# RozDavid/UnScene3D

Hardware: AMD Instinct MI355X
Metric: training scenes/sec (Res16UNet34C+Mask3D, 150k voxels) (higher is better)
Workload: dtype f32

## Files before the change

include/usc3d.h:

```cpp
#ifndef USC3D_H
#define USC3D_H

#include <stdint.h>

#ifdef __cplusplus
extern "C" {
#endif

typedef void* usc_stream_t;

enum usc_status {
  USC_OK = 0,
  USC_ERR_ARG = -1,
  USC_ERR_LAUNCH = -2,
  USC_ERR_RANGE = -3
};

const char* usc_last_error(void);
int usc_abi_version(void);
const char* usc_build_info(void);
int usc_device_count(void);


int usc_voxel_floor_f64(const double* xyz, int64_t n, double voxel_size,
                        int32_t* coords_out, usc_stream_t s);

int usc_voxel_floor_f64_host(const double* xyz, int64_t n, double voxel_size,
                             int32_t* coords_out);
int usc_unique_coords_host(const int32_t* coords, int64_t n, int32_t d,
                           int64_t* unique_idx, int64_t* inverse,
                           int64_t* n_out);

int64_t usc_coordmap_capacity(int64_t n);
int64_t usc_coordmap_ws_bytes(int64_t n);

int usc_coordmap_build(const int32_t* coords, int64_t n, int32_t quant,
                       uint64_t* table_keys, int32_t* table_vals, int64_t cap,
                       int64_t* unique_idx, int64_t* inverse,
                       int32_t* out_coords, int64_t* n_out,
                       void* ws, int64_t ws_bytes, usc_stream_t s);

int usc_morton_cell_ids(const int32_t* coords, int64_t n, int32_t shift,
                        int32_t lo_x, int32_t lo_y, int32_t lo_z,
                        int32_t bits_per_axis, int64_t* ids, usc_stream_t s);


int usc_kernel_map_cube(const int32_t* coords, int64_t n, int32_t tensor_stride,
                        int32_t ksize, const uint64_t* table_keys,
                        const int32_t* table_vals, int64_t cap, int32_t* nbr,
                        usc_stream_t s);

int usc_kernel_map_down2(const int32_t* fine_coords, int64_t n_fine,
                         int32_t tensor_stride, const int64_t* parent,
                         const int32_t* coarse_coords, int64_t n_coarse,
                         int32_t* nbr2, uint8_t* kidx, usc_stream_t s);

int64_t usc_rulebook_ws_bytes(int64_t K, int64_t n_out);
int usc_rulebook_compact(const int32_t* nbr, int64_t K, int64_t n_out,
                         int32_t* in_idx, int32_t* out_idx, int64_t* koff,
                         void* ws, int64_t ws_bytes, usc_stream_t s);


int usc_weight_transpose(const float* W, int32_t K, int32_t cin, int32_t cout,
                         int32_t mirror, float* out, usc_stream_t s);

int usc_spconv_plan(int32_t kind, int64_t n, int32_t cin, int32_t cout,
                    int32_t K);
int64_t usc_rowsort_ws_bytes(int32_t K, int64_t n_out);
int usc_rowsort_build(const int32_t* nbr, int32_t K, int64_t n_out,
                      int32_t* perm, uint32_t* tile_mask, void* ws,
                      int64_t ws_bytes, usc_stream_t s);
int64_t usc_spconv_sorted_ws_bytes(int64_t n_out, int32_t cin, int32_t cout,
                                   int32_t K);
int usc_spconv_sorted_gemm(const float* in, int64_t n_in, int32_t cin,
                           const float* W, int32_t K, int32_t cout,
                           const int32_t* nbr, const int32_t* perm,
                           const uint32_t* tile_mask, int64_t n_out,
                           const float* bias, float* out, int32_t accumulate,
                           int32_t w_transposed, void* ws, int64_t ws_bytes,
                           usc_stream_t s);
int usc_spconv_sorted_gemm_ex(const float* in, int64_t n_in, int32_t cin,
                              const float* W, int32_t K, int32_t cout,
                              const int32_t* nbr, const int32_t* perm,
                              const uint32_t* tile_mask, int64_t n_out,
                              const float* bias, float* out, int32_t accumulate,
                              int32_t w_transposed, void* ws, int64_t ws_bytes,
                              int32_t* slices_left, usc_stream_t s);
int usc_group_reduce(const float* partial, int32_t G, int64_t n, int32_t c,
                     const float* bias, int32_t accumulate, float* out,
                     usc_stream_t s);

int64_t usc_spconv_gather_gemm_ws_bytes(int64_t n_out, int32_t cin,
                                        int32_t cout, int32_t K);
int usc_spconv_gather_gemm(const float* in, int64_t n_in, int32_t cin,
                           const float* W, int32_t K, int32_t cout,
                           const int32_t* nbr, int64_t n_out,
                           const float* bias, float* out, int32_t accumulate, int32_t w_transposed,
                           void* ws, int64_t ws_bytes, usc_stream_t s);

int usc_spconv_pairs_gemm(const float* in, int32_t cin, const float* W,
                          int32_t K, int32_t cout, const int32_t* rows_in,
                          const int32_t* rows_out, const int64_t* koff,
                          int64_t P_capacity, float* out, usc_stream_t s);

int usc_cast_bf16(const float* in, int64_t n, uint16_t* out, usc_stream_t s);
int usc_spconv_pack_w_bf16(const float* W, int32_t K, int32_t cin, int32_t cout,
                           uint16_t* Wp, usc_stream_t s);
int64_t usc_spconv_gather_gemm_bf16_ws_bytes(int64_t n_out, int32_t cin,
                                             int32_t cout, int32_t K);
int usc_spconv_gather_gemm_bf16(const uint16_t* in, int64_t n_in, int32_t cin,
                                const uint16_t* Wp, int32_t K, int32_t cout,
                                const int32_t* nbr, int64_t n_out,
                                const float* bias, float* out, int32_t accumulate,
                                void* ws, int64_t ws_bytes, usc_stream_t s);

int usc_split_bf16_rows(const float* in, int64_t rows, int32_t c, int32_t P,
                        uint16_t* out, usc_stream_t s);
int usc_split_bf16(const float* in, int64_t n, int32_t P, uint16_t* out,
                   usc_stream_t s);
int usc_spconv_pack_w_split(const float* W, int32_t K, int32_t cin, int32_t cout,
// ... 477 lines not shown
```

unscene3d_amd/_lib.py:

```python
from __future__ import annotations

import ctypes as C
import os

import torch

_HERE = os.path.dirname(os.path.abspath(__file__))
LIB_PATH = os.environ.get("USC3D_LIB") or os.path.join(_HERE, "libusc3d_hip.so")

_p = C.c_void_p
_i32 = C.c_int32
_i64 = C.c_int64
_f64 = C.c_double
_f32 = C.c_float

class KMap(C.Structure):
    _fields_ = [("nbr", _p), ("perm", _p), ("tile_mask", _p), ("pair_in", _p), ("pair_out", _p), ("koff", _p),
                ("n_in", _i64), ("n_out", _i64), ("pair_capacity", _i64), ("K", _i32), ("reserved", _i32)]


class BNDesc(C.Structure):
    _fields_ = [("gamma", _p), ("beta", _p), ("running_mean", _p), ("running_var", _p), ("num_batches_tracked", _p),
                ("eps", _f32), ("momentum", _f32), ("c", _i32), ("training", _i32)]


_kp = C.POINTER(KMap)
_bp = C.POINTER(BNDesc)


class Step(C.Structure):
    _fields_ = [("op", _i32), ("kind", _i32), ("cin", _i32), ("cout", _i32), ("relu", _i32),
                ("dx_accumulate", _i32), ("dW_accumulate", _i32), ("dbn_accumulate", _i32), ("defer_wgrad", _i32),
                ("accumulate", _i32),
                ("map", _p), ("bn", _p),
                ("x", _p), ("W", _p), ("residual", _p), ("y", _p), ("stats", _p), ("out", _p),
                ("dout", _p), ("dy", _p), ("dres", _p), ("dx", _p), ("dW", _p), ("dgamma", _p), ("dbeta", _p),
                ("a", _p), ("b", _p), ("dst", _p), ("dst2", _p), ("n", _i64), ("ca", _i32), ("cb", _i32),
                ("split_planes", _i32), ("reserved", _i32)]


_sp = C.POINTER(Step)
STEP_UNIT_FWD, STEP_UNIT_BWD, STEP_CAT, STEP_SPLIT, STEP_ADD, STEP_UNIT_FWD_BF16 = 0, 1, 2, 3, 4, 5

SIGNATURES = {
    "usc_last_error": (C.c_char_p, []),
    "usc_abi_version": (C.c_int, []),
    "usc_build_info": (C.c_char_p, []),
    "usc_device_count": (C.c_int, []),
    "usc_voxel_floor_f64": (C.c_int, [_p, _i64, _f64, _p, _p]),
    "usc_voxel_floor_f64_host": (C.c_int, [_p, _i64, C.c_double, _p]),
    "usc_unique_coords_host": (C.c_int, [_p, _i64, _i32, _p, _p, _p]),
    "usc_coordmap_capacity": (_i64, [_i64]),
    "usc_coordmap_ws_bytes": (_i64, [_i64]),
    "usc_coordmap_build": (C.c_int, [_p, _i64, _i32, _p, _p, _i64, _p, _p, _p, _p, _p, _i64, _p]),
    "usc_morton_cell_ids": (C.c_int, [_p, _i64, _i32, _i32, _i32, _i32, _i32, _p, _p]),
    "usc_kernel_map_cube": (C.c_int, [_p, _i64, _i32, _i32, _p, _p, _i64, _p, _p]),
    "usc_kernel_map_down2": (C.c_int, [_p, _i64, _i32, _p, _p, _i64, _p, _p, _p]),
    "usc_rulebook_ws_bytes": (_i64, [_i64, _i64]),
    "usc_rulebook_compact": (C.c_int, [_p, _i64, _i64, _p, _p, _p, _p, _i64, _p]),
    "usc_weight_transpose": (C.c_int, [_p, _i32, _i32, _i32, _i32, _p, _p]),
    "usc_spconv_plan": (C.c_int, [_i32, _i64, _i32, _i32, _i32]),
    "usc_spconv_gather_gemm_ws_bytes": (_i64, [_i64, _i32, _i32, _i32]),
    "usc_spconv_gather_gemm": (C.c_int, [_p, _i64, _i32, _p, _i32, _i32, _p, _i64, _p, _p, _i32, _i32, _p, _i64, _p]),
    "usc_rowsort_ws_bytes": (_i64, [_i32, _i64]),
    "usc_rowsort_build": (C.c_int, [_p, _i32, _i64, _p, _p, _p, _i64, _p]),
    "usc_spconv_sorted_ws_bytes": (_i64, [_i64, _i32, _i32, _i32]),
    "usc_spconv_sorted_gemm": (C.c_int, [_p, _i64, _i32, _p, _i32, _i32, _p, _p, _p, _i64, _p, _p, _i32, _i32, _p, _i64, _p]),
    "usc_spconv_sorted_gemm_ex": (C.c_int, [_p, _i64, _i32, _p, _i32, _i32, _p, _p, _p, _i64, _p, _p, _i32, _i32, _p, _i64, _p, _p]),
    "usc_group_reduce": (C.c_int, [_p, _i32, _i64, _i32, _p, _i32, _p, _p]),
    "usc_bn_tile_max_rows": (C.c_int64, []),
    "usc_bn_plan": (_i64, [_i64, _i32, _i32]),
    "usc_bn_tile_ok": (C.c_int, [_i64, _i32]),
    "usc_bn_tile_ws_bytes": (C.c_int64, [_i32]),
    "usc_bn_tile_forward": (C.c_int, [_p, _i32, _p, _i64, _i32, _p, _p, _f32, _f32, _p, _p, _p, _p, _p, _p, _p, _p, _i32, _p,
                                      _p, _i64, _p]),
    "usc_bn_tile_backward": (C.c_int, [_p, _i32, _i32, _p, _p, _p, _p, _p, _p, _i64, _i32, _i32, _i32, _p, _p, _p, _p, _p,
                                       _i64, _p]),
    "usc_spconv_pairs_gemm": (C.c_int, [_p, _i32, _p, _i32, _i32, _p, _p, _p, _i64, _p, _p]),
    "usc_cast_bf16": (C.c_int, [_p, _i64, _p, _p]),
    "usc_spconv_pack_w_bf16": (C.c_int, [_p, _i32, _i32, _i32, _p, _p]),
    "usc_spconv_gather_gemm_bf16_ws_bytes": (_i64, [_i64, _i32, _i32, _i32]),
    "usc_spconv_gather_gemm_bf16": (C.c_int, [_p, _i64, _i32, _p, _i32, _i32, _p, _i64, _p, _p, _i32, _p, _i64, _p]),
    "usc_split_bf16_rows": (C.c_int, [_p, _i64, _i32, _i32, _p, _p]),
    "usc_split_bf16": (C.c_int, [_p, _i64, _i32, _p, _p]),
    "usc_spconv_pack_w_split": (C.c_int, [_p, _i32, _i32, _i32, _i32, _i32, _p, _p]),
    "usc_spconv_gather_gemm_split_ws_bytes": (_i64, [_i64, _i32, _i32, _i32, _i32]),
    "usc_spconv_gather_gemm_split": (C.c_int, [_p, _i64, _i32, _p, _i32, _i32, _i32, _p, _i64, _p, _p, _i32, _p, _i64, _p]),
    "usc_spconv_wgrad_ws_bytes": (_i64, [_i32, _i32, _i32]),
    "usc_spconv_wgrad": (C.c_int, [_p, _i32, _p, _i32, _i32, _p, _p, _p, _i64, _p, _i32, _p, _i64, _p]),
    "usc_spconv_wgrad_ws_bytes_rows": (_i64, [_i32, _i32, _i32, _i64]),
    "usc_step_size": (_i32, []),
    "usc_program_ws_bytes": (_i64, [_sp, _i32]),
    "usc_program_run": (C.c_int, [_sp, _i32, _i32, _p, _i64, _p]),
    "usc_spconv_wgrad_group_max": (_i32, []),
    "usc_spconv_wgrad_grid_limit": (None, [_i32]),
    "usc_spconv_wgrad_group_ok": (C.c_int, [_i32, _i32, _i32, _i32, _i64]),
    "usc_spconv_wgrad_group": (C.c_int, [_i32, _p, _p, _p, _i32, _i32, _i32, _p, _p, _p, _i64, _i32, _p]),
    "usc_spconv_wgrad_table_ws_bytes": (_i64, [_i32, _i32, _i32]),
    "usc_spconv_wgrad_table": (C.c_int, [_p, _i32, _p, _i32, _p, _i32, _i64, _p, _i32, _p, _i64, _p]),
    "usc_set_wgrad_lane": (C.c_int, [_p, _p, _i64, _i64]),
    "usc_wgrad_lane_join": (C.c_int, [_p]),
    "usc_wgrad_lane_hold": (C.c_int, [_i32, _i64, _i64, _p]),
    "usc_wgrad_lane_holding": (_i32, []),
    "usc_launch_stats_begin": (C.c_int, [_p, _i64, _p]),
    "usc_launch_stats_end": (_i64, [_p, _i64]),
    "usc_wall_clock_khz": (_i64, []),
    "usc_conv_ws_bytes": (_i64, [_kp, _i32, _i32, _i32]),
    "usc_unit_ws_bytes": (_i64, [_kp, _i32, _i32, _i32]),
    "usc_conv_forward": (C.c_int, [_kp, _i32, _p, _i32, _p, _i32, _p, _p, _p, _i64, _p]),
    "usc_conv_backward": (C.c_int, [_kp, _i32, _p, _i32, _p, _i32, _p, _p, _i32, _p, _i32, _p, _i64, _p]),
    "usc_bn_eval_stats": (C.c_int, [_p, _p, _p, _p, _f32, _i32, _p, _p, _p, _p, _p]),
    "usc_conv_bn_act_forward": (C.c_int, [_kp, _i32, _p, _i32, _p, _i32, _bp, _p, _i32, _p, _p, _p, _p, _i64, _p]),
    "usc_unit_bf16_ws_bytes": (_i64, [_kp, _i32, _i32, _i32]),
    "usc_conv_bn_act_forward_bf16": (C.c_int, [_kp, _i32, _p, _i32, _p, _i32, _bp, _p, _i32, _p, _p, _p, _p, _i64, _p]),
    "usc_unit_split_ws_bytes": (_i64, [_kp, _i32, _i32, _i32, _i32]),
    "usc_conv_bn_act_forward_split": (C.c_int, [_kp, _i32, _p, _i32, _p, _i32, _i32, _bp, _p, _i32, _p, _p, _p, _p, _i64, _p]),
# ... 144 lines not shown
```

unscene3d_amd/csrc/common.h:

```cpp
#pragma once
#include <hip/hip_runtime.h>
#include <stdint.h>
#include <stdio.h>
#include <string.h>

#include "../../include/usc3d.h"

namespace usc {

constexpr int kWave = 64;

void set_error(const char* fmt, ...);

#define USC_REQUIRE(cond, ...)                   \
  do {                                           \
    if (!(cond)) {                               \
      ::usc::set_error(__VA_ARGS__);             \
      return USC_ERR_ARG;                        \
    }                                            \
  } while (0)

#define USC_CHECK_LAUNCH(name)                                                  \
  do {                                                                          \
    hipError_t e__ = hipGetLastError();                                         \
// ... 35 lines not shown
  k ^= k >> 30; k *= 0xbf58476d1ce4e5b9ull;
  k ^= k >> 27; k *= 0x94d049bb133111ebull;
  k ^= k >> 31;
  return k;
}

__host__ __device__ inline int floor_quant(int c, int q) {
  int d = c / q;
  if ((c % q != 0) && ((c < 0) != (q < 0))) --d;
  return d * q;
}

#if defined(__HIPCC__)
__device__ inline int table_lookup(const uint64_t* __restrict__ keys,
                                   const int32_t* __restrict__ vals, int64_t cap,
                                   uint64_t key) {
  uint64_t slot = hash_key(key) & (uint64_t)(cap - 1);
  for (;;) {
    uint64_t k = keys[slot];
    if (k == key) return vals[slot];
    if (k == kEmptyKey) return -1;
    slot = (slot + 1) & (uint64_t)(cap - 1);
  }
}

__device__ inline int lane_id() { return threadIdx.x & 63; }

__device__ inline int wave_reduce_add(int v) {
#pragma unroll
  for (int o = 32; o > 0; o >>= 1) v += __shfl_xor(v, o, 64);
  return v;
}
__device__ inline float wave_reduce_addf(float v) {
#pragma unroll
  for (int o = 32; o > 0; o >>= 1) v += __shfl_xor(v, o, 64);
  return v;
}
__device__ inline double wave_reduce_addd(double v) {
#pragma unroll
  for (int o = 32; o > 0; o >>= 1) v += __shfl_xor(v, o, 64);
  return v;
}
__device__ inline int wave_inclusive_scan(int v) {
  const int l = lane_id();
#pragma unroll
  for (int o = 1; o < 64; o <<= 1) {
    int t = __shfl_up(v, o, 64);
    if (l >= o) v += t;
  }
  return v;
}
#endif

int spconv_up_table(const int32_t* nbr2, int32_t K, int64_t n_coarse, int64_t n_fine, int32_t* inv, hipStream_t st);

}
```

unscene3d_amd/csrc/spconv.hip:

```cpp
#include "common.h"

#include <stdlib.h>

#include <vector>

namespace usc {

typedef float f32x16 __attribute__((ext_vector_type(16)));

#define MFMA32(a, b, c) __builtin_amdgcn_mfma_f32_32x32x2f32((a), (b), (c), 0, 0, 0)

struct GemmParams {
  const float* in;
  const float* W;
  const int32_t* nbr;
  const float* bias;
  float* out;
  int64_t n_out;
  int cin, cout, K;
  int accumulate;
  int G;
  int TM;
  int wt1;
  const int32_t* rows_in;
// ... 891 lines not shown
  const int64_t total = per * K;
  for (int64_t j = (int64_t)blockIdx.x * blockDim.x + threadIdx.x; j < total; j += (int64_t)gridDim.x * blockDim.x) {
    const int k = (int)(j / per);
    const int64_t rem = j - (int64_t)k * per;
    const int co = (int)(rem / cin), ci = (int)(rem - (int64_t)co * cin);
    const int ks = mirror ? (K - 1 - k) : k;
    out[j] = W[(int64_t)ks * per + (int64_t)ci * cout + co];
  }
}

__global__ void weight_pack_kernel(const float* __restrict__ W, int K, int cin, int cout, int NB, int wt,
                                   float* __restrict__ out) {
  const int64_t total = (int64_t)K * cin * cout;
  const int nq = cin >> 3, BN = NB * 32;
  for (int64_t e = (int64_t)blockIdx.x * blockDim.x + threadIdx.x; e < total; e += (int64_t)gridDim.x * blockDim.x) {
    int64_t r = e;
    const int j = (int)(r & 3); r >>= 2;
    const int ln = (int)(r & 63); r >>= 6;
    const int nb = (int)(r % NB); r /= NB;
    const int q = (int)(r % nq); r /= nq;
    const int k = (int)(r % K);
    const int cb = (int)(r / K);
    const int i = ln & 31, h = ln >> 5;
    const int c = 8 * q + 4 * h + j, n = cb * BN + NB * i + nb;
    out[e] = wt ? W[((int64_t)(K - 1 - k) * cout + n) * cin + c] : W[((int64_t)k * cin + c) * cout + n];
  }
}

static int wgrad_splits(int K, int cin, int cout, int NB, int64_t n_rows) {
  const int64_t tiles = (int64_t)K * ceil_div(cin, 32) * ceil_div(cout, NB * 32);
  const int target = (K > 1 && n_rows >= (int64_t)2 << 20) ? 4096 : 2048;
  int64_t S = ceil_div(target, tiles);
  const int64_t by_rows = n_rows / 2048 + 1;
  if (S > by_rows) S = by_rows;
  if (S > 64) S = 64;
  if (S < 1) S = 1;
  return (int)S;
}
static int wgrad_full_nb(int cb) { return (cb % 3 == 0) ? 3 : (cb % 4 == 0 ? 4 : (cb % 2 == 0 ? 2 : 1)); }
static int wgrad_full_ct(int ctiles, int NBf) {
  if (NBf == 3 && ctiles % 3 != 0 && ctiles % 4 == 0) return 4;
  return (ctiles % 3 == 0 && NBf * 3 <= 9) ? 3 : ((ctiles % 4 == 0 && NBf * 4 <= 9) ? 4 : ((ctiles % 2 == 0 && NBf * 2 <= 9) ? 2 : 1));
}
static int64_t wgrad_full_splits(int K, int ctiles, int cb, int CT, int NBf, int64_t n_rows) {
  const int64_t blocks_per_split = (int64_t)K * (ctiles / CT) * (cb / NBf);
  const int64_t tgt = (K > 1 && n_rows >= (int64_t)2 << 20) ? 2048 : 512;
  int64_t S = tgt / blocks_per_split;
  const int64_t by_rows = n_rows / (K > 1 ? 4096 : 256) + 1;
  if (S > by_rows) S = by_rows;
  if (S > 64) S = 64;
  if (S < 1) S = 1;
  return S;
}
static int pick_nb(int cout) {
  if (cout <= 32) return 1;
  if (cout <= 64) return 2;
  if (cout % 128 == 0) return 4;
  if (cout % 96 == 0) return 3;
  return 4;
}

struct GemmPlan { int NB; int G; bool aligned; int TM; };
constexpr int64_t kTargetWaves = 3072;

static bool stem_form(bool has_table, int cin, int cout, int K) {
  return has_table && cin >= 1 && cin <= 4 && cout == 32 && K >= 1 && K <= 32;
}

static GemmPlan plan_table(int64_t n_out, int cin, int cout, int K) {
  GemmPlan pl{pick_nb(cout), 1, false, 0};
  const bool al = (cin % 32 == 0) && (cout % 32 == 0);
  if (!al) return pl;
  pl.aligned = true;
  if (K > 1 && K <= kMaxK && n_out >= 24576 && cin >= 64 && cin <= kZeroRowFloats) {
    const int cb = cout / 32;
    const int nb = (cb % 3 == 0) ? 3 : (cb % 2 == 0 ? 2 : 1);
    constexpr int kTmMax3 = 192;
    constexpr int64_t kTileSlots = 256;
    const int tm_max = nb == 3 ? kTmMax3 : 256;
    int64_t R = 1;
    int64_t tm = ceil_div(n_out, kTileSlots * R);
    while (tm > tm_max) { ++R; tm = ceil_div(n_out, kTileSlots * R); }
    tm = (tm + 3) & ~3ll;
    pl.NB = nb;
    pl.TM = (int)tm;
    return pl;
  }
  const int64_t row_tiles = ceil_div(n_out, 32);
  const int cb = cout / 32;
  const int cands[4] = {4, 3, 2, 1};
  int chosen = 1;
  for (int c = 0; c < 4; ++c) {
    const int nb = cands[c];
    if (cb % nb) continue;
    if (row_tiles * (cb / nb) >= kTargetWaves) { chosen = nb; break; }
  }
  pl.NB = chosen;
  const int64_t waves = row_tiles * (cb / chosen);
  if (waves > 0 && waves < kTargetWaves && K > 1) {
    int64_t G = ceil_div(kTargetWaves, waves);
    if (G > K) G = K;
    pl.G = (int)G;
  }
  return pl;
}
static GemmPlan plan_list(int64_t max_tiles, int cin, int cout) {
  GemmPlan pl{pick_nb(cout), 1, false, 0};
  const bool al = (cin % 32 == 0) && (cout % 32 == 0);
  if (!al) return pl;
  pl.aligned = true;
  const int cb = cout / 32;
  const int cands[4] = {4, 3, 2, 1};
  int chosen = 1;
  for (int c = 0; c < 4; ++c) {
    const int nb = cands[c];
    if (cb % nb) continue;
    if (max_tiles * (cb / nb) >= kTargetWaves) { chosen = nb; break; }
  }
  pl.NB = chosen;
  return pl;
}

template <bool LIST>
static void launch_gemm(const GemmPlan& pl, dim3 grid, hipStream_t st, const GemmParams& p) {
#define USC_GG(NBv)                                                                                      \
  if (pl.aligned && p.wt1)        \
    hipLaunchKernelGGL((gather_gemm_aligned_kernel<NBv, false, true>), grid, dim3(256), 0, st, p);      \
  else if (pl.aligned)                                                                                   \
    hipLaunchKernelGGL((gather_gemm_aligned_kernel<NBv, LIST>), grid, dim3(256), 0, st, p);             \
  else                                                                                                   \
    hipLaunchKernelGGL((gather_gemm_kernel<NBv, LIST>), grid, dim3(256), 0, st, p);
  switch (pl.NB) {
    case 1: USC_GG(1) break;
    case 2: USC_GG(2) break;
    case 3: USC_GG(3) break;
    default: USC_GG(4) break;
  }
#undef USC_GG
}

}

using namespace usc;

extern "C" {

int usc_weight_transpose(const float* W, int32_t K, int32_t cin, int32_t cout, int32_t mirror, float* out,
                         usc_stream_t s) {
  USC_REQUIRE(W && out && K >= 1 && cin >= 1 && cout >= 1, "usc_weight_transpose: bad argument");
  const int64_t total = (int64_t)K * cin * cout;
  hipLaunchKernelGGL(weight_transpose_kernel, dim3(stream_grid(total, 256)), dim3(256), 0, as_stream(s), W, (int)K,
                     (int)cin, (int)cout, (int)mirror, out);
  USC_CHECK_LAUNCH("usc_weight_transpose");
  return USC_OK;
}

int usc_spconv_plan(int32_t kind, int64_t n, int32_t cin, int32_t cout, int32_t K) {
  GemmPlan pl;
  if (kind == 0 && stem_form(K > 1, cin, cout, K)) return 1 | (1 << 14);
  if (kind == 0) pl = plan_table(n, cin, cout, K);
  else if (kind == 1) pl = plan_list(ceil_div(n, 32) + K, cin, cout);
  else {
    const int ctiles = cin / 32, cb = cout / 32;
    const int NBf = (cb % 3 == 0) ? 3 : (cb % 4 == 0 ? 4 : (cb % 2 == 0 ? 2 : 1));
    if (cin % 32 == 0 && cout % 32 == 0 && (!(NBf == 3 && ctiles % 3 != 0) || ctiles % 4 == 0)) {
      const int CT = wgrad_full_ct(ctiles, NBf);
      return NBf | (1 << 8) | (1 << 13) | (CT << 16);
    }
    const int NB = pick_nb(cout);
    pl = GemmPlan{NB, 1, (cin % 32 == 0) && (cout % (NB * 32) == 0), 0};
  }
  return pl.NB | ((pl.aligned ? 1 : 0) << 8) | ((pl.TM > 0 ? 1 : 0) << 12) | (pl.G << 16);
}

int64_t usc_spconv_gather_gemm_ws_bytes(int64_t n_out, int32_t cin, int32_t cout, int32_t K) {
  const GemmPlan pl = plan_table(n_out, cin, cout, K);
  if (pl.TM > 0) return (int64_t)K * cin * cout * 4;
  return pl.G > 1 ? (int64_t)pl.G * n_out * cout * 4 : 0;
}

namespace {
struct LaunchStats { unsigned long long* ring = nullptr; int64_t slots = 0, count = 0; std::vector<usc_launch_stat> meta; };
LaunchStats g_lstats;
__global__ void launch_stats_init_kernel(unsigned long long* ring, int64_t slots) {
  const int64_t i = (int64_t)blockIdx.x * blockDim.x + threadIdx.x;
  if (i < slots) { ring[4 * i] = ~0ull; ring[4 * i + 1] = 0; ring[4 * i + 2] = 0; ring[4 * i + 3] = 0; }
}
}

int usc_launch_stats_begin(void* ring_dev, int64_t slots, usc_stream_t s) {
  USC_REQUIRE(ring_dev && slots > 0, "usc_launch_stats_begin: needs a device ring of slots x 4 x u64");
  hipLaunchKernelGGL(launch_stats_init_kernel, dim3((unsigned)ceil_div(slots, 256)), dim3(256), 0, as_stream(s),
                     (unsigned long long*)ring_dev, slots);
  USC_CHECK_LAUNCH("usc_launch_stats_begin");
  g_lstats.ring = (unsigned long long*)ring_dev;
  g_lstats.slots = slots;
  g_lstats.count = 0;
  g_lstats.meta.clear();
  g_lstats.meta.reserve((size_t)slots);
  return USC_OK;
}

int64_t usc_launch_stats_end(usc_launch_stat* host_out, int64_t max_out) {
  const int64_t n = g_lstats.count;
  if (host_out)
    for (int64_t i = 0; i < n && i < max_out; ++i) host_out[i] = g_lstats.meta[(size_t)i];
  g_lstats.ring = nullptr;
  g_lstats.slots = g_lstats.count = 0;
  g_lstats.meta.clear();
  return n;
}

int64_t usc_wall_clock_khz(void) {
  int dev = 0, khz = 0;
  if (hipGetDevice(&dev) != hipSuccess || hipDeviceGetAttribute(&khz, hipDeviceAttributeWallClockRate, dev) != hipSuccess) return 0;
  return khz;
}

int usc_spconv_gather_gemm(const float* in, int64_t n_in, int32_t cin, const float* W, int32_t K, int32_t cout,
                           const int32_t* nbr, int64_t n_out, const float* bias, float* out, int32_t accumulate,
                           int32_t w_transposed, void* ws, int64_t ws_bytes, usc_stream_t s) {
  USC_REQUIRE(cin >= 1 && cout >= 1 && K >= 1 && n_out >= 0 && n_in >= 0, "usc_spconv_gather_gemm: bad sizes");
  USC_REQUIRE(nbr || K == 1, "usc_spconv_gather_gemm: K>1 needs a neighbour table");
  USC_REQUIRE(nbr || n_in == n_out, "usc_spconv_gather_gemm: identity map needs n_in == n_out");
  if (n_out == 0) return USC_OK;
  USC_REQUIRE(in && W && out, "usc_spconv_gather_gemm: null pointer");
  if (stem_form(nbr != nullptr, cin, cout, K) && !accumulate && !w_transposed) {
    hipLaunchKernelGGL(stem_conv_kernel, dim3((unsigned)ceil_div(n_out, 256)), dim3(256), 0, as_stream(s), in, W, nbr, bias,
                       out, n_out, (int)K, (int)cin);
    USC_CHECK_LAUNCH("usc_spconv_gather_gemm");
    return USC_OK;
  }
  const GemmPlan pl = plan_table(n_out, cin, cout, K);
  GemmParams p{};
  p.in = in; p.W = W; p.nbr = nbr; p.bias = bias; p.out = out;
  p.n_out = n_out; p.cin = cin; p.cout = cout; p.K = K; p.accumulate = accumulate; p.G = pl.G;
  if (pl.G > 1) {
    USC_REQUIRE(ws && ws_bytes >= (int64_t)pl.G * n_out * cout * 4, "usc_spconv_gather_gemm: workspace too small");
    p.out = (float*)ws;
  }
  hipStream_t st = as_stream(s);
  const bool wt1 = w_transposed && K == 1 && !nbr && pl.aligned && pl.TM == 0;
  USC_REQUIRE(!w_transposed || pl.TM > 0 || wt1,
              "usc_spconv_gather_gemm: w_transposed is only folded into the tile-compacted kernel (usc_spconv_plan bit 12) "
              "and, for K = 1 on identity rows with channel counts in multiples of 32, into the row-order kernel; "
              "use usc_weight_transpose for other shapes");
  p.wt1 = wt1 ? 1 : 0;
  if (pl.TM > 0) {
    p.TM = pl.TM;
    USC_REQUIRE(ws && ws_bytes >= (int64_t)K * cin * cout * 4, "usc_spconv_gather_gemm: workspace too small");
    hipLaunchKernelGGL(weight_pack_kernel, dim3(stream_grid((int64_t)K * cin * cout, 256)), dim3(256), 0, st, W, (int)K,
                       (int)cin, (int)cout, pl.NB, (int)w_transposed, (float*)ws);
    p.W = (const float*)ws;
    dim3 cgrid((unsigned)ceil_div(n_out, pl.TM), (unsigned)(cout / (pl.NB * 32)));
    const size_t lds = compact_lds_bytes(pl.NB, pl.TM);
    if (g_lstats.ring && g_lstats.count < g_lstats.slots) {
      p.stats = g_lstats.ring + 4 * g_lstats.count++;
      g_lstats.meta.push_back(usc_launch_stat{n_out, cin, cout, K, pl.NB});
    }
#define USC_CG(NBv)                                                                                        \
    {                                                                                                      \
      static bool attr_set = false;                                                                        \
      auto kfn = gather_gemm_compact_kernel<NBv>;                                                          \
      if (!attr_set) {                                                                                     \
        (void)hipFuncSetAttribute((const void*)kfn, hipFuncAttributeMaxDynamicSharedMemorySize, 160 * 1024); \
        attr_set = true;                                                                                   \
      }                                                                                                    \
      hipLaunchKernelGGL(kfn, cgrid, dim3(64 * kCompactWaves), lds, st, p);                                \
    }
    if (pl.NB == 3) USC_CG(3) else if (pl.NB == 2) USC_CG(2) else USC_CG(1)
#undef USC_CG
    USC_CHECK_LAUNCH("usc_spconv_gather_gemm");
    return USC_OK;
  }
  dim3 grid((unsigned)ceil_div(n_out, 128), (unsigned)ceil_div(cout, pl.NB * 32), (unsigned)pl.G);
  launch_gemm<false>(pl, grid, st, p);
  if (pl.G > 1) {
    const int64_t numel4 = n_out * cout / 4;
    hipLaunchKernelGGL(group_reduce_kernel, dim3(stream_grid(numel4, 256)), dim3(256), 0, st, (const float*)ws, pl.G,
                       numel4, (int)cout, bias, (int)accumulate, out);
  }
  USC_CHECK_LAUNCH("usc_spconv_gather_gemm");
  return USC_OK;
}

int usc_spconv_pairs_gemm(const float* in, int32_t cin, const float* W, int32_t K, int32_t cout,
                          const int32_t* rows_in, const int32_t* rows_out, const int64_t* koff, int64_t P_capacity,
                          float* out, usc_stream_t s) {
  USC_REQUIRE(cin >= 1 && cout >= 1 && K >= 1 && P_capacity >= 0, "usc_spconv_pairs_gemm: bad sizes");
  if (P_capacity == 0) return USC_OK;
  USC_REQUIRE(in && W && rows_in && rows_out && koff && out, "usc_spconv_pairs_gemm: null pointer");
  GemmParams p{};
  p.in = in; p.W = W; p.out = out; p.cin = cin; p.cout = cout; p.K = K; p.G = 1;
  p.rows_in = rows_in; p.rows_out = rows_out; p.koff = koff;
  const int64_t max_tiles = ceil_div(P_capacity, 32) + K;
  const GemmPlan pl = plan_list(max_tiles, cin, cout);
  dim3 grid((unsigned)ceil_div(max_tiles, 4), (unsigned)ceil_div(cout, pl.NB * 32));
  launch_gemm<true>(pl, grid, as_stream(s), p);
  USC_CHECK_LAUNCH("usc_spconv_pairs_gemm");
  return USC_OK;
}

int64_t usc_spconv_wgrad_ws_bytes(int32_t K, int32_t cin, int32_t cout) {
  return (int64_t)64 * K * cin * cout * (int64_t)sizeof(float);
}

int64_t usc_spconv_wgrad_ws_bytes_rows(int32_t K, int32_t cin, int32_t cout, int64_t n_rows) {
  const int64_t numel = (int64_t)K * cin * cout;
  const int ctiles = cin / 32, cb = cout / 32;
  if (cin % 32 == 0 && cout % 32 == 0 && cb > 0) {
    const int NBf = wgrad_full_nb(cb);
    if (!(NBf == 3 && ctiles % 3 != 0) || ctiles % 4 == 0)
      return wgrad_full_splits(K, ctiles, cb, wgrad_full_ct(ctiles, NBf), NBf, n_rows) * numel * 4;
  }
  return (int64_t)wgrad_splits(K, cin, cout, pick_nb(cout), n_rows) * numel * 4;
}

int64_t usc_spconv_wgrad_table_ws_bytes(int32_t K, int32_t cin, int32_t cout) {
  return (int64_t)kStemSplits * K * cin * cout * 4;
}

int usc_spconv_wgrad_table(const float* in, int32_t cin, const float* dy, int32_t cout, const int32_t* nbr, int32_t K,
                           int64_t n_out, float* dW, int32_t accumulate, void* ws, int64_t ws_bytes, usc_stream_t s) {
  USC_REQUIRE(cin >= 1 && cin <= 4 && cout == 32 && K >= 1 && K <= 32 && n_out >= 0,
              "usc_spconv_wgrad_table: the table form covers <= 4 input channels and 32 output channels (the stem)");
  USC_REQUIRE(in && dy && nbr && dW && ws, "usc_spconv_wgrad_table: null pointer");
  USC_REQUIRE(ws_bytes >= usc_spconv_wgrad_table_ws_bytes(K, cin, cout), "usc_spconv_wgrad_table: workspace too small");
  hipStream_t st = as_stream(s);
  const int per = 32 / cin, groups = (K + per - 1) / per;
  const int64_t numel = (int64_t)K * cin * 32;
  hipLaunchKernelGGL(stem_wgrad_kernel, dim3(kStemSplits, (unsigned)groups), dim3(64 * kStemWaves), 0, st, in, dy, nbr, n_out, (int)K,
                     (int)cin, (float*)ws);
  hipLaunchKernelGGL(wgrad_reduce_kernel, dim3(stream_grid(numel, 256)), dim3(256), 0, st, (const float*)ws, kStemSplits, numel,
                     (int)accumulate, dW);
  USC_CHECK_LAUNCH("usc_spconv_wgrad_table");
  return USC_OK;
}

static int g_wgrad_grid_limit = 0;
void usc_spconv_wgrad_grid_limit(int32_t max_workgroups) { g_wgrad_grid_limit = max_workgroups; }

int usc_spconv_wgrad(const float* a, int32_t cin, const float* b, int32_t cout, int32_t K, const int32_t* a_idx,
                     const int32_t* b_idx, const int64_t* koff, int64_t n_rows, float* dW, int32_t accumulate, void* ws, int64_t ws_bytes,
                     usc_stream_t s) {
  USC_REQUIRE(cin >= 1 && cout >= 1 && K >= 1 && n_rows >= 0, "usc_spconv_wgrad: bad sizes");
  USC_REQUIRE(a && b && dW && ws, "usc_spconv_wgrad: null pointer");
  USC_REQUIRE((a_idx && b_idx && koff) || (!a_idx && K == 1), "usc_spconv_wgrad: pair lists required for K>1");
  const int64_t numel = (int64_t)K * cin * cout;
  hipStream_t st = as_stream(s);
  WgradParams p{};
  p.a = a; p.b = b; p.a_idx = a_idx; p.b_idx = b_idx; p.koff = koff; p.n_rows = n_rows;
  p.partial = (float*)ws; p.cin = cin; p.cout = cout; p.K = K;
  const int ctiles = cin / 32, cb = cout / 32;
  const int NBf = wgrad_full_nb(cb);
  if (cin % 32 == 0 && cout % 32 == 0 && (!(NBf == 3 && ctiles % 3 != 0) || ctiles % 4 == 0)) {
    const int CT = wgrad_full_ct(ctiles, NBf);
    const int64_t S = wgrad_full_splits(K, ctiles, cb, CT, NBf, n_rows);
    USC_REQUIRE(ws_bytes >= S * numel * 4, "usc_spconv_wgrad: workspace too small");
    p.S = (int)S;
    if (S == 1) { p.direct = dW; p.accumulate = accumulate; }
    dim3 grid((unsigned)(K * S), (unsigned)(ctiles / CT), (unsigned)(cb / NBf));
    if (g_wgrad_grid_limit > 0 && (int64_t)K * S > g_wgrad_grid_limit) {
      p.vblocks = (int)(K * S);
      grid.x = (unsigned)g_wgrad_grid_limit;
    }
    const size_t lds = (size_t)4 * NBf * 16 * 64 * sizeof(float);
#define USC_WF(C, N) if (CT == C && NBf == N) { \
      static bool attr_set = false; auto kfn = wgrad_full_kernel<C, N>; \
      if (!attr_set) { (void)hipFuncSetAttribute((const void*)kfn, hipFuncAttributeMaxDynamicSharedMemorySize, 64 * 1024); attr_set = true; } \
      hipLaunchKernelGGL(kfn, grid, dim3(256), lds, st, p, WgradGroup{}); }
    USC_WF(3, 3) USC_WF(2, 3) USC_WF(1, 3) USC_WF(2, 4) USC_WF(1, 4) USC_WF(4, 2) USC_WF(3, 2) USC_WF(2, 2) USC_WF(1, 2) USC_WF(4, 1) USC_WF(3, 1) USC_WF(2, 1) USC_WF(1, 1)
    USC_WF(4, 3)
#undef USC_WF
    if (S > 1)
      hipLaunchKernelGGL(wgrad_reduce_kernel, dim3(stream_grid(numel, 256)), dim3(256), 0, st, (const float*)ws, (int)S,
                         numel, (int)accumulate, dW);
    USC_CHECK_LAUNCH("usc_spconv_wgrad");
    return USC_OK;
  }
  const int NB = pick_nb(cout);
  const bool aligned = (cin % 32 == 0) && (cout % (NB * 32) == 0);
  const int S = wgrad_splits(K, cin, cout, NB, n_rows);
  USC_REQUIRE(ws_bytes >= (int64_t)S * numel * 4, "usc_spconv_wgrad: workspace too small");
  p.S = S;
  dim3 grid((unsigned)(K * S), (unsigned)ceil_div(cin, 32), (unsigned)ceil_div(cout, NB * 32));
  const size_t lds = (size_t)3 * NB * 16 * 64 * sizeof(float);
#define USC_WG(NBv)                                                                          \
  if (aligned) hipLaunchKernelGGL((wgrad_kernel<NBv, true>), grid, dim3(256), lds, st, p);  \
  else hipLaunchKernelGGL((wgrad_kernel<NBv, false>), grid, dim3(256), lds, st, p);
  switch (NB) {
    case 1: USC_WG(1) break;
    case 2: USC_WG(2) break;
    case 3: USC_WG(3) break;
    default: USC_WG(4) break;
  }
#undef USC_WG
  hipLaunchKernelGGL(wgrad_reduce_kernel, dim3(stream_grid(numel, 256)), dim3(256), 0, st, (const float*)ws, S, numel,
                     (int)accumulate, dW);
  USC_CHECK_LAUNCH("usc_spconv_wgrad");
  return USC_OK;
}

int32_t usc_spconv_wgrad_group_max(void) { return kMaxWgradGroup; }

int usc_spconv_wgrad_group_ok(int32_t R, int32_t cin, int32_t cout, int32_t K, int64_t n_rows) {
// ... 46 lines not shown
```

Measured before the change: 43.99.

## Add dense MFMA GEMM path for 1x1 sparse convolutions and their weight gradients

Adds a dedicated dense GEMM kernel using fp32 MFMA 32x32x2 instructions with double-buffered LDS staging. It is used for K=1 (no neighbour map) convolution forward passes and for weight gradients when the sizes qualify, in place of the generic gather-GEMM and wgrad kernels. The tile and split-K plan is chosen from the row count and channel widths, and split partials are reduced with the existing reduce kernel. The aim is to avoid the indirection overhead on pointwise layers. This adds a new code path that is on by default and can be turned off with an environment variable.

```diff
diff --git a/include/usc3d.h b/include/usc3d.h
--- a/include/usc3d.h
+++ b/include/usc3d.h
@@ -66,6 +66,7 @@
 
 int usc_spconv_plan(int32_t kind, int64_t n, int32_t cin, int32_t cout,
                     int32_t K);
+int usc_dense_plan(int32_t form, int64_t n, int32_t cin, int32_t cout);
 int64_t usc_rowsort_ws_bytes(int32_t K, int64_t n_out);
 int usc_rowsort_build(const int32_t* nbr, int32_t K, int64_t n_out,
                       int32_t* perm, uint32_t* tile_mask, void* ws,
diff --git a/unscene3d_amd/_lib.py b/unscene3d_amd/_lib.py
--- a/unscene3d_amd/_lib.py
+++ b/unscene3d_amd/_lib.py
@@ -60,8 +60,9 @@
     "usc_rulebook_compact": (C.c_int, [_p, _i64, _i64, _p, _p, _p, _p, _i64, _p]),
     "usc_weight_transpose": (C.c_int, [_p, _i32, _i32, _i32, _i32, _p, _p]),
     "usc_spconv_plan": (C.c_int, [_i32, _i64, _i32, _i32, _i32]),
+    "usc_dense_plan": (C.c_int, [_i32, _i64, _i32, _i32]),
     "usc_spconv_gather_gemm_ws_bytes": (_i64, [_i64, _i32, _i32, _i32]),
-    "usc_spconv_gather_gemm": (C.c_int, [_p, _i64, _i32, _p, _i32, _i32, _p, _i64, _p, _p, _i32, _i32, _p, _i64, _p]),
+    "usc_spconv_gather_gemm":(C.c_int, [_p, _i64, _i32, _p, _i32, _i32, _p, _i64, _p, _p, _i32, _i32, _p, _i64, _p]),
     "usc_rowsort_ws_bytes": (_i64, [_i32, _i64]),
     "usc_rowsort_build": (C.c_int, [_p, _i32, _i64, _p, _p, _p, _i64, _p]),
     "usc_spconv_sorted_ws_bytes": (_i64, [_i64, _i32, _i32, _i32]),
diff --git a/unscene3d_amd/csrc/common.h b/unscene3d_amd/csrc/common.h
--- a/unscene3d_amd/csrc/common.h
+++ b/unscene3d_amd/csrc/common.h
@@ -111,6 +111,14 @@
 }
 #endif
 
+struct DensePlan { int bm, bn, S; };
+DensePlan dense_plan(int form, int64_t n, int cin, int cout);
+bool dense_k1_enabled();
+void dense_gemm_launch(const float* in, int64_t n, int cin, const float* W, int cout, const float* bias, float* out,
+                       int accumulate, int w_transposed, hipStream_t st);
+void dense_wgrad_launch(const float* a, int cin, const float* b, int cout, int64_t n, float* dst, int accumulate,
+                        int grid_limit, hipStream_t st);
+
 int spconv_up_table(const int32_t* nbr2, int32_t K, int64_t n_coarse, int64_t n_fine, int32_t* inv, hipStream_t st);
 
 }
diff --git a/unscene3d_amd/csrc/dense.hip b/unscene3d_amd/csrc/dense.hip
--- /dev/null
+++ b/unscene3d_amd/csrc/dense.hip
@@ -0,0 +1,291 @@
+#include "common.h"
+
+#include <stdlib.h>
+
+namespace usc {
+
+typedef float f32x16 __attribute__((ext_vector_type(16)));
+
+enum { kDenseNN = 0, kDenseNT = 1, kDenseTN = 2 };
+
+struct DenseParams {
+  const float* A;
+  const float* B;
+  const float* bias;
+  float* C;
+  int64_t n;
+  int cin, cout;
+  int accumulate;
+  int S;
+  int64_t L;
+  int vblocks;
+};
+
+__device__ inline int dense_acc_row(int reg, int half) { return (reg & 3) + 8 * (reg >> 2) + 4 * half; }
+
+template <int MT, int NT, int WM, int WN, int BK, int D, int MODE>
+__global__ __launch_bounds__(64 * WM * WN) void dense_gemm_kernel(DenseParams p) {
+  constexpr int BM = 32 * MT * WM, BN = 32 * NT * WN, NTHR = 64 * WM * WN;
+  constexpr bool A_KMAJOR = MODE == kDenseTN, B_KMAJOR = MODE != kDenseNT;
+  constexpr int A_FLOATS = A_KMAJOR ? BK * BM : BM * (BK + 1);
+  constexpr int B_FLOATS = B_KMAJOR ? BK * BN : BN * (BK + 1);
+  constexpr int A_PAD = (A_FLOATS + 3) & ~3, B_PAD = (B_FLOATS + 3) & ~3;
+  constexpr int A_V4 = BM * BK / 4, B_V4 = BN * BK / 4;
+  constexpr int A_PER = (A_V4 + NTHR - 1) / NTHR, B_PER = (B_V4 + NTHR - 1) / NTHR;
+  __shared__ __attribute__((aligned(16))) float As[2][A_PAD];
+  __shared__ __attribute__((aligned(16))) float Bs[2][B_PAD];
+
+  const int tid = threadIdx.x, lane = tid & 63, wave = tid >> 6;
+  const int i = lane & 31, h = lane >> 5;
+  const int wm0 = (wave / WN) * (32 * MT), wn0 = (wave % WN) * (32 * NT);
+  const int cin = p.cin, cout = p.cout;
+  const int n0 = blockIdx.y * BN;
+  const int vtotal = MODE == kDenseTN ? p.vblocks : (int)gridDim.x;
+
+  for (int vb = blockIdx.x; vb < vtotal; vb += gridDim.x) {
+    int64_t m0, r_begin, r_end;
+    int s = 0;
+    if (MODE == kDenseTN) {
+      const int mtiles = cin / BM;
+      const int grp = vb / (8 * mtiles), within = vb - grp * (8 * mtiles);
+      const int gs = p.S - 8 * grp < 8 ? p.S - 8 * grp : 8;
+      s = 8 * grp + within % gs;
+      m0 = (int64_t)(within / gs) * BM;
+      r_begin = (int64_t)s * p.L;
+      r_end = r_begin + p.L < p.n ? r_begin + p.L : p.n;
+    } else {
+      m0 = (int64_t)vb * BM;
+      r_begin = 0;
+      r_end = cin;
+    }
+
+    f32x16 acc[MT][NT];
+#pragma unroll
+    for (int mt = 0; mt < MT; ++mt)
+#pragma unroll
+      for (int nt = 0; nt < NT; ++nt)
+#pragma unroll
+        for (int r = 0; r < 16; ++r) acc[mt][nt][r] = 0.f;
+
+    const int64_t nslab = (r_end - r_begin + BK - 1) / BK;
+    float4 ra[D][A_PER], rb[D][B_PER];
+    auto fetch = [&](const int slot, int64_t t) {
+      const int64_t r0 = r_begin + t * BK;
+      const bool live = t < nslab;
+#pragma unroll
+      for (int u = 0; u < A_PER; ++u) {
+        const int idx = tid + u * NTHR;
+        float4 v = make_float4(0.f, 0.f, 0.f, 0.f);
+        if (live && (A_V4 % NTHR == 0 || idx < A_V4)) {
+          if (A_KMAJOR) {
+            const int k = idx / (BM / 4), c4 = idx - k * (BM / 4);
+            if (r0 + k < r_end) v = *reinterpret_cast<const float4*>(p.A + (r0 + k) * cin + m0 + 4 * c4);
+          } else {
+            const int x = idx / (BK / 4), c4 = idx - x * (BK / 4);
+            if (m0 + x < p.n) v = *reinterpret_cast<const float4*>(p.A + (m0 + x) * cin + r0 + 4 * c4);
+          }
+        }
+        ra[slot][u] = v;
+      }
+#pragma unroll
+      for (int u = 0; u < B_PER; ++u) {
+        const int idx = tid + u * NTHR;
+        float4 v = make_float4(0.f, 0.f, 0.f, 0.f);
+        if (live && (B_V4 % NTHR == 0 || idx < B_V4)) {
+          if (B_KMAJOR) {
+            const int k = idx / (BN / 4), c4 = idx - k * (BN / 4);
+            if (r0 + k < r_end) v = *reinterpret_cast<const float4*>(p.B + (r0 + k) * cout + n0 + 4 * c4);
+          } else {
+            const int x = idx / (BK / 4), c4 = idx - x * (BK / 4);
+            v = *reinterpret_cast<const float4*>(p.B + (int64_t)(n0 + x) * cin + r0 + 4 * c4);
+          }
+        }
+        rb[slot][u] = v;
+      }
+    };
+    auto stage = [&](const int slot, const int b) {
+#pragma unroll
+      for (int u = 0; u < A_PER; ++u) {
+        const int idx = tid + u * NTHR;
+        if (A_V4 % NTHR == 0 || idx < A_V4) {
+          if (A_KMAJOR) {
+            *reinterpret_cast<float4*>(&As[b][4 * idx]) = ra[slot][u];
+          } else {
+            const int x = idx / (BK / 4), c4 = idx - x * (BK / 4);
+            float* d = &As[b][x * (BK + 1) + 4 * c4];
+            d[0] = ra[slot][u].x; d[1] = ra[slot][u].y; d[2] = ra[slot][u].z; d[3] = ra[slot][u].w;
+          }
+        }
+      }
+#pragma unroll
+      for (int u = 0; u < B_PER; ++u) {
+        const int idx = tid + u * NTHR;
+        if (B_V4 % NTHR == 0 || idx < B_V4) {
+          if (B_KMAJOR) {
+            *reinterpret_cast<float4*>(&Bs[b][4 * idx]) = rb[slot][u];
+          } else {
+            const int x = idx / (BK / 4), c4 = idx - x * (BK / 4);
+            float* d = &Bs[b][x * (BK + 1) + 4 * c4];
+            d[0] = rb[slot][u].x; d[1] = rb[slot][u].y; d[2] = rb[slot][u].z; d[3] = rb[slot][u].w;
+          }
+        }
+      }
+    };
+
+    constexpr int U = (D % 2 == 0) ? D : 2 * D;
+    fetch(0, 0);
+    stage(0, 0);
+#pragma unroll
+    for (int u = 1; u <= D; ++u) fetch(u % D, u);
+    __syncthreads();
+    for (int64_t t0 = 0; t0 < nslab; t0 += U) {
+#pragma unroll
+      for (int u = 0; u < U; ++u) {
+        const int64_t t = t0 + u;
+        if (t >= nslab) break;
+        const float* as = As[u & 1];
+        const float* bs = Bs[u & 1];
+#pragma unroll
+        for (int q = 0; q < BK / 2; ++q) {
+          const int k = 2 * q + h;
+          float av[MT], bv[NT];
+#pragma unroll
+          for (int mt = 0; mt < MT; ++mt)
+            av[mt] = A_KMAJOR ? as[k * BM + wm0 + 32 * mt + i] : as[(wm0 + 32 * mt + i) * (BK + 1) + k];
+#pragma unroll
+          for (int nt = 0; nt < NT; ++nt)
+            bv[nt] = B_KMAJOR ? bs[k * BN + wn0 + 32 * nt + i] : bs[(wn0 + 32 * nt + i) * (BK + 1) + k];
+#pragma unroll
+          for (int mt = 0; mt < MT; ++mt)
+#pragma unroll
+            for (int nt = 0; nt < NT; ++nt)
+              acc[mt][nt] = __builtin_amdgcn_mfma_f32_32x32x2f32(av[mt], bv[nt], acc[mt][nt], 0, 0, 0);
+        }
+        if (t + 1 < nslab) stage((u + 1) % D, (u + 1) & 1);
+        fetch((u + 1) % D, t + 1 + D);
+        __syncthreads();
+      }
+    }
+
+    const int64_t m_end = MODE == kDenseTN ? (int64_t)cin : p.n;
+    float* cbase = p.C;
+    bool rmw = p.accumulate != 0;
+    if (MODE == kDenseTN && p.S > 1) {
+      cbase += (int64_t)s * cin * cout;
+      rmw = false;
+    }
+#pragma unroll
+    for (int mt = 0; mt < MT; ++mt)
+#pragma unroll
+      for (int r = 0; r < 16; ++r) {
+        const int64_t row = m0 + wm0 + 32 * mt + dense_acc_row(r, h);
+        if (row >= m_end) continue;
+#pragma unroll
+        for (int nt = 0; nt < NT; ++nt) {
+          const int col = n0 + wn0 + 32 * nt + i;
+          float v = acc[mt][nt][r];
+          float* dst = cbase + row * cout + col;
+          if (MODE != kDenseTN && p.bias) v += p.bias[col];
+          if (rmw) v += *dst;
+          *dst = v;
+        }
+      }
+  }
+}
+
+constexpr int64_t kDenseCUs = 256;
+
+static int dense_width(int cout, int at_most) {
+  const int cb = cout / 32;
+  for (int w = at_most; w > 1; --w)
+    if (cb % w == 0) return w;
+  return 1;
+}
+
+DensePlan dense_plan(int form, int64_t n, int cin, int cout) {
+  DensePlan pl{};
+  if (form == kDenseTN) {
+    pl.bm = 32;
+    pl.bn = 32 * dense_width(cout, 4);
+    const int64_t tiles = (int64_t)(cin / 32) * (cout / pl.bn);
+    int64_t S = (4 * kDenseCUs + tiles - 1) / tiles;
+    const int64_t by_rows = n / 256 + 1;
+    if (S > by_rows) S = by_rows;
+    if (S > 64) S = 64;
+    if (S < 1) S = 1;
+    pl.S = (int)S;
+    return pl;
+  }
+  pl.S = 1;
+  const int wide = cout % 128 == 0 ? 4 : dense_width(cout, 3);
+  const int bigm = wide == 4 ? 64 : 128;
+  const int64_t big = ((n + bigm - 1) / bigm) * (cout / (32 * wide));
+  if (big >= kDenseCUs * (bigm == 64 ? 2 : 1)) {
+    pl.bm = bigm;
+    pl.bn = 32 * wide;
+    return pl;
+  }
+  pl.bm = 32;
+  const int64_t row_tiles = (n + 31) / 32;
+  int w = dense_width(cout, 4);
+  while (w > 1 && row_tiles * (cout / (32 * w)) < kDenseCUs) w = dense_width(cout, w - 1);
+  pl.bn = 32 * w;
+  return pl;
+}
+
+bool dense_k1_enabled() {
+  static const int on = [] {
+    const char* e = getenv("USC3D_DENSE_K1");
+    return (e && e[0] == '0' && e[1] == 0) ? 0 : 1;
+  }();
+  return on != 0;
+}
+
+template <int MODE>
+static void dense_launch_mode(const DensePlan& pl, dim3 grid, hipStream_t st, const DenseParams& p) {
+#define USC_DG(MT, NT, WM, WN, BK, D) \
+  hipLaunchKernelGGL((dense_gemm_kernel<MT, NT, WM, WN, BK, D, MODE>), grid, dim3(64 * WM * WN), 0, st, p)
+  if (pl.bm == 64) {
+    USC_DG(1, 2, 2, 2, 16, 3);
+  } else if (pl.bm == 128) {
+    switch (pl.bn) {
+      case 96: USC_DG(1, 3, 4, 1, 16, 1); break;
+      case 64: USC_DG(1, 2, 4, 1, 16, 1); break;
+      default: USC_DG(1, 1, 4, 1, 16, 1); break;
+    }
+  } else {
+    switch (pl.bn) {
+      case 128: USC_DG(1, 1, 1, 4, 32, 1); break;
+      case 96: USC_DG(1, 1, 1, 3, 32, 1); break;
+      case 64: USC_DG(1, 1, 1, 2, 32, 1); break;
+      default: USC_DG(1, 1, 1, 1, 32, 1); break;
+    }
+  }
+#undef USC_DG
+}
+
+void dense_gemm_launch(const float* in, int64_t n, int cin, const float* W, int cout, const float* bias, float* out,
+                       int accumulate, int w_transposed, hipStream_t st) {
+  const DensePlan pl = dense_plan(w_transposed ? kDenseNT : kDenseNN, n, cin, cout);
+  DenseParams p{};
+  p.A = in; p.B = W; p.bias = bias; p.C = out; p.n = n; p.cin = cin; p.cout = cout; p.accumulate = accumulate; p.S = 1;
+  dim3 grid((unsigned)((n + pl.bm - 1) / pl.bm), (unsigned)(cout / pl.bn));
+  if (w_transposed) dense_launch_mode<kDenseNT>(pl, grid, st, p);
+  else dense_launch_mode<kDenseNN>(pl, grid, st, p);
+}
+
+void dense_wgrad_launch(const float* a, int cin, const float* b, int cout, int64_t n, float* dst, int accumulate,
+                        int grid_limit, hipStream_t st) {
+  const DensePlan pl = dense_plan(kDenseTN, n, cin, cout);
+  DenseParams p{};
+  p.A = a; p.B = b; p.C = dst; p.n = n; p.cin = cin; p.cout = cout; p.accumulate = accumulate; p.S = pl.S;
+  int64_t L = (n + pl.S - 1) / pl.S;
+  p.L = (L + 31) / 32 * 32;
+  if (p.L < 32) p.L = 32;
+  p.vblocks = pl.S * (cin / 32);
+  dim3 grid((unsigned)p.vblocks, (unsigned)(cout / pl.bn));
+  if (grid_limit > 0 && p.vblocks > grid_limit) grid.x = (unsigned)grid_limit;
+  dense_launch_mode<kDenseTN>(pl, grid, st, p);
+}
+
+}
diff --git a/unscene3d_amd/csrc/spconv.hip b/unscene3d_amd/csrc/spconv.hip
--- a/unscene3d_amd/csrc/spconv.hip
+++ b/unscene3d_amd/csrc/spconv.hip
@@ -967,6 +967,18 @@
   if (S < 1) S = 1;
   return S;
 }
+static bool dense_form(int cin, int cout) { return cin >= 32 && cout >= 32 && cin % 32 == 0 && cout % 32 == 0; }
+static bool dense_fwd_takes(int64_t n, int cin, int cout) { return dense_form(cin, cout) && n >= 2048; }
+static bool dense_wgrad_takes(int64_t n, int cin, int cout) {
+  if (!dense_form(cin, cout) || n < 32768) return false;
+  const int ctiles = cin / 32, cb = cout / 32, NBf = wgrad_full_nb(cb);
+  if (NBf == 3 && ctiles % 3 != 0 && ctiles % 4 != 0) return false;
+  const int CT = wgrad_full_ct(ctiles, NBf);
+  const DensePlan dp = dense_plan(2, n, cin, cout);
+  if ((int64_t)dp.S * ctiles * (cout / dp.bn) < 256) return false;
+  return wgrad_full_splits(1, ctiles, cb, CT, NBf, n) * (ctiles / CT) * (cb / NBf) < 128;
+}
+
 static int pick_nb(int cout) {
   if (cout <= 32) return 1;
   if (cout <= 64) return 2;
@@ -1073,6 +1085,7 @@
 int usc_spconv_plan(int32_t kind, int64_t n, int32_t cin, int32_t cout, int32_t K) {
   GemmPlan pl;
   if (kind == 0 && stem_form(K > 1, cin, cout, K)) return 1 | (1 << 14);
+  const int dense = (K == 1 && dense_k1_enabled() && ((kind == 0 && dense_fwd_takes(n, cin, cout)) || (kind == 2 && dense_wgrad_takes(n, cin, cout)))) ? (1 << 15) : 0;
   if (kind == 0) pl = plan_table(n, cin, cout, K);
   else if (kind == 1) pl = plan_list(ceil_div(n, 32) + K, cin, cout);
   else {
@@ -1080,12 +1093,19 @@
     const int NBf = (cb % 3 == 0) ? 3 : (cb % 4 == 0 ? 4 : (cb % 2 == 0 ? 2 : 1));
     if (cin % 32 == 0 && cout % 32 == 0 && (!(NBf == 3 && ctiles % 3 != 0) || ctiles % 4 == 0)) {
       const int CT = wgrad_full_ct(ctiles, NBf);
-      return NBf | (1 << 8) | (1 << 13) | (CT << 16);
+      return NBf | (1 << 8) | (1 << 13) | (CT << 16) | dense;
     }
     const int NB = pick_nb(cout);
     pl = GemmPlan{NB, 1, (cin % 32 == 0) && (cout % (NB * 32) == 0), 0};
   }
-  return pl.NB | ((pl.aligned ? 1 : 0) << 8) | ((pl.TM > 0 ? 1 : 0) << 12) | (pl.G << 16);
+  return dense | pl.NB | ((pl.aligned ? 1 : 0) << 8) | ((pl.TM > 0 ? 1 : 0) << 12) | (pl.G << 16);
+}
+
+int usc_dense_plan(int32_t form, int64_t n, int32_t cin, int32_t cout) {
+  if (form < 0 || form > 2 || n < 0 || cin < 32 || cout < 32 || cin % 32 || cout % 32) return 0;
+  const DensePlan pl = dense_plan(form, n, cin, cout);
+  const bool taken = form == 2 ? dense_wgrad_takes(n, cin, cout) : dense_fwd_takes(n, cin, cout);
+  return pl.bm | (pl.bn << 8) | (pl.S << 16) | ((taken ? 1 : 0) << 29) | ((dense_k1_enabled() ? 1 : 0) << 30);
 }
 
 int64_t usc_spconv_gather_gemm_ws_bytes(int64_t n_out, int32_t cin, int32_t cout, int32_t K) {
@@ -1143,6 +1163,11 @@
   if (stem_form(nbr != nullptr, cin, cout, K) && !accumulate && !w_transposed) {
     hipLaunchKernelGGL(stem_conv_kernel, dim3((unsigned)ceil_div(n_out, 256)), dim3(256), 0, as_stream(s), in, W, nbr, bias,
                        out, n_out, (int)K, (int)cin);
+    USC_CHECK_LAUNCH("usc_spconv_gather_gemm");
+    return USC_OK;
+  }
+  if (!nbr && K == 1 && dense_k1_enabled() && dense_fwd_takes(n_out, cin, cout)) {
+    dense_gemm_launch(in, n_out, (int)cin, W, (int)cout, bias, out, (int)accumulate, (int)w_transposed, as_stream(s));
     USC_CHECK_LAUNCH("usc_spconv_gather_gemm");
     return USC_OK;
   }
@@ -1223,12 +1248,15 @@
 int64_t usc_spconv_wgrad_ws_bytes_rows(int32_t K, int32_t cin, int32_t cout, int64_t n_rows) {
   const int64_t numel = (int64_t)K * cin * cout;
   const int ctiles = cin / 32, cb = cout / 32;
-  if (cin % 32 == 0 && cout % 32 == 0 && cb > 0) {
+  const int64_t dense_S = (K == 1 && dense_k1_enabled() && dense_wgrad_takes(n_rows, cin, cout)) ? dense_plan(2, n_rows, cin, cout).S : 0;
+  int64_t S;
+  if (cin % 32 == 0 && cout % 32 == 0 && cb > 0 && (!(wgrad_full_nb(cb) == 3 && ctiles % 3 != 0) || ctiles % 4 == 0)) {
     const int NBf = wgrad_full_nb(cb);
-    if (!(NBf == 3 && ctiles % 3 != 0) || ctiles % 4 == 0)
-      return wgrad_full_splits(K, ctiles, cb, wgrad_full_ct(ctiles, NBf), NBf, n_rows) * numel * 4;
-  }
-  return (int64_t)wgrad_splits(K, cin, cout, pick_nb(cout), n_rows) * numel * 4;
+    S = wgrad_full_splits(K, ctiles, cb, wgrad_full_ct(ctiles, NBf), NBf, n_rows);
+  } else {
+    S = wgrad_splits(K, cin, cout, pick_nb(cout), n_rows);
+  }
+  return (S > dense_S ? S : dense_S) * numel * 4;
 }
 
 int64_t usc_spconv_wgrad_table_ws_bytes(int32_t K, int32_t cin, int32_t cout) {
@@ -1266,6 +1294,16 @@
   WgradParams p{};
   p.a = a; p.b = b; p.a_idx = a_idx; p.b_idx = b_idx; p.koff = koff; p.n_rows = n_rows;
   p.partial = (float*)ws; p.cin = cin; p.cout = cout; p.K = K;
+  if (!a_idx && K == 1 && dense_k1_enabled() && dense_wgrad_takes(n_rows, cin, cout)) {
+    const int S = dense_plan(2, n_rows, cin, cout).S;
+    USC_REQUIRE(S == 1 || ws_bytes >= (int64_t)S * numel * 4, "usc_spconv_wgrad: workspace too small");
+    dense_wgrad_launch(a, (int)cin, b, (int)cout, n_rows, S == 1 ? dW : (float*)ws, (int)accumulate, g_wgrad_grid_limit, st);
+    if (S > 1)
+      hipLaunchKernelGGL(wgrad_reduce_kernel, dim3(stream_grid(numel, 256)), dim3(256), 0, st, (const float*)ws, S,
+                         numel, (int)accumulate, dW);
+    USC_CHECK_LAUNCH("usc_spconv_wgrad");
+    return USC_OK;
+  }
   const int ctiles = cin / 32, cb = cout / 32;
   const int NBf = wgrad_full_nb(cb);
   if (cin % 32 == 0 && cout % 32 == 0 && (!(NBf == 3 && ctiles % 3 != 0) || ctiles % 4 == 0)) {
```

Result: no change. 44.01 (median of 2 runs) (+0.1%).
